# DarylFernandes99/custom-yolo-implmentation

Hardware: AMD Instinct MI355X
Metric: images/sec (640x640 bf16) (higher is better)
Workload: dtype bf16; 1 GPU; preset s (width 32..512, depth 1) 640x640 train step (fwd+DFL/QFL loss+bwd+grad sync+AdamW), COCO-80 synthetic, 32 img/GPU; global_batch=32, parallelism=dp1, hip_graph=True, optimizer_in_graph=True, deterministic_mode=False

## Files before the change

custom-yolo-implmentation_amd/csrc/elementwise.hip:

```cpp
#include "common.h"

namespace {

constexpr int TPB = 256;
constexpr int RS_ROWS = 2;
constexpr int RS_MAXBLK = 256 * 8;

template <typename T> __host__ bool vec_ok(const void* p, long ld, int C) {
    constexpr int V = vec_of<T>::N;
    return (C % V == 0) && (ld % V == 0) && ((reinterpret_cast<uintptr_t>(p) % 16) == 0);
}

template <typename TI, typename TO>
__global__ void k_ncm_to_nhwc(const TI* __restrict__ src, long sn, long sc, long off,
                              TO* __restrict__ dst, int ld, int C, int HW) {
    __shared__ float tile[32][33];
    const int n = blockIdx.z, p0 = blockIdx.x * 32, c0 = blockIdx.y * 32;
    const int tx = threadIdx.x & 31, ty = threadIdx.x >> 5;
    for (int r = ty; r < 32; r += 8) {
        int c = c0 + r, p = p0 + tx;
        tile[r][tx] = (c < C && p < HW) ? to_f<TI>(src[n * sn + c * sc + off + p]) : 0.f;
    }
    __syncthreads();
    for (int r = ty; r < 32; r += 8) {
        int p = p0 + r, c = c0 + tx;
        if (p < HW && c < C) dst[((long)n * HW + p) * ld + c] = from_f<TO>(tile[tx][r]);
    }
}

template <typename TI, typename TO>
__global__ void k_nhwc_to_ncm(const TI* __restrict__ src, int ld, TO* __restrict__ dst, long sn,
                              long sc, long off, int C, int HW) {
    __shared__ float tile[32][33];
    const int n = blockIdx.z, p0 = blockIdx.x * 32, c0 = blockIdx.y * 32;
    const int tx = threadIdx.x & 31, ty = threadIdx.x >> 5;
    for (int r = ty; r < 32; r += 8) {
        int p = p0 + r, c = c0 + tx;
        tile[r][tx] = (p < HW && c < C) ? to_f<TI>(src[((long)n * HW + p) * ld + c]) : 0.f;
    }
    __syncthreads();
    for (int r = ty; r < 32; r += 8) {
        int c = c0 + r, p = p0 + tx;
        if (c < C && p < HW) dst[n * sn + c * sc + off + p] = from_f<TO>(tile[tx][r]);
    }
}

constexpr int HEAD_GROUP = 8;
struct HeadGroup {
    void* t[HEAD_GROUP];
    int ld[HEAD_GROUP], C[HEAD_GROUP], HW[HEAD_GROUP], c_off[HEAD_GROUP], m_off[HEAD_GROUP], tp[HEAD_GROUP];
    int start[HEAD_GROUP + 1];
    int n;
};

template <typename T, bool PACK>
__global__ __launch_bounds__(256) void k_head_group(HeadGroup g, T* __restrict__ preds, long sn, long sc) {
    __shared__ float tile[32][33];
    int bi = 0;
#pragma unroll
    for (int i = 1; i < HEAD_GROUP; ++i)
        if (i < g.n && (int)blockIdx.x >= g.start[i]) bi = i;
    T* x; int ld, C, HW, c_off, m_off, tp, st;
#define HG_PICK(I) case I: x = (T*)g.t[I]; ld = g.ld[I]; C = g.C[I]; HW = g.HW[I]; c_off = g.c_off[I]; m_off = g.m_off[I]; tp = g.tp[I]; st = g.start[I]; break;
    switch (bi) {
        HG_PICK(1) HG_PICK(2) HG_PICK(3) HG_PICK(4) HG_PICK(5) HG_PICK(6) HG_PICK(7)
        default: x = (T*)g.t[0]; ld = g.ld[0]; C = g.C[0]; HW = g.HW[0]; c_off = g.c_off[0]; m_off = g.m_off[0]; tp = g.tp[0]; st = g.start[0]; break;
    }
#undef HG_PICK
    const int tl = (int)blockIdx.x - st;
    const int n = blockIdx.y, p0 = (tl % tp) * 32, c0 = (tl / tp) * 32;
    const int tx = threadIdx.x & 31, ty = threadIdx.x >> 5;
    T* pr = preds + n * sn + (long)c_off * sc + m_off;
    if (PACK) {
        for (int r = ty; r < 32; r += 8) {
            const int p = p0 + r, c = c0 + tx;
            tile[r][tx] = (p < HW && c < C) ? to_f<T>(x[((long)n * HW + p) * ld + c]) : 0.f;
        }
        __syncthreads();
        for (int r = ty; r < 32; r += 8) {
            const int c = c0 + r, p = p0 + tx;
            if (c < C && p < HW) pr[c * sc + p] = from_f<T>(tile[tx][r]);
        }
    } else {
        for (int r = ty; r < 32; r += 8) {
            const int c = c0 + r, p = p0 + tx;
            tile[r][tx] = (c < C && p < HW) ? to_f<T>(pr[c * sc + p]) : 0.f;
        }
        __syncthreads();
        for (int r = ty; r < 32; r += 8) {
            const int p = p0 + r, c = c0 + tx;
            if (p < HW && c < C) x[((long)n * HW + p) * ld + c] = from_f<T>(tile[tx][r]);
        }
    }
}

template <typename T, bool PACK>
__global__ __launch_bounds__(256) void k_head_group_vec(HeadGroup g, T* __restrict__ preds, long sn, long sc) {
    extern __shared__ __attribute__((aligned(16))) unsigned char hg_raw[];
    T* tile = reinterpret_cast<T*>(hg_raw);
    int bi = 0;
#pragma unroll
    for (int i = 1; i < HEAD_GROUP; ++i)
        if (i < g.n && (int)blockIdx.x >= g.start[i]) bi = i;
    T* x; int ld, C, HW, c_off, m_off, st;
#define HG_PICK(I) case I: x = (T*)g.t[I]; ld = g.ld[I]; C = g.C[I]; HW = g.HW[I]; c_off = g.c_off[I]; m_off = g.m_off[I]; st = g.start[I]; break;
    switch (bi) {
        HG_PICK(1) HG_PICK(2) HG_PICK(3) HG_PICK(4) HG_PICK(5) HG_PICK(6) HG_PICK(7)
        default: x = (T*)g.t[0]; ld = g.ld[0]; C = g.C[0]; HW = g.HW[0]; c_off = g.c_off[0]; m_off = g.m_off[0]; st = g.start[0]; break;
    }
#undef HG_PICK
    const int n = blockIdx.y, p0 = ((int)blockIdx.x - st) * 64;
    const int LDT = C + 2, cpr = C / 8;
    T* pr = preds + n * sn + (long)c_off * sc + m_off;
    T* xr = x + ((long)n * HW + p0) * ld;
    const int npx = HW - p0 < 64 ? HW - p0 : 64;
    if (PACK) {
        for (int i = threadIdx.x; i < npx * cpr; i += 256) {
            const int p = i / cpr, ch = (i - p * cpr) * 8;
            const pack_t<T, 8> v = load_raw<T, 8>(xr + (long)p * ld + ch);
#pragma unroll
            for (int e = 0; e < 8; ++e) tile[p * LDT + ch + e] = v.v[e];
        }
        __syncthreads();
        for (int i = threadIdx.x; i < C * (npx / 8); i += 256) {
            const int c = i / (npx / 8), pg = (i - c * (npx / 8)) * 8;
            pack_t<T, 8> v;
#pragma unroll
            for (int e = 0; e < 8; ++e) v.v[e] = tile[(pg + e) * LDT + c];
            *reinterpret_cast<pack_t<T, 8>*>(pr + c * sc + p0 + pg) = v;
        }
    } else {
        for (int i = threadIdx.x; i < C * (npx / 8); i += 256) {
            const int c = i / (npx / 8), pg = (i - c * (npx / 8)) * 8;
            const pack_t<T, 8> v = load_raw<T, 8>(pr + c * sc + p0 + pg);
#pragma unroll
            for (int e = 0; e < 8; ++e) tile[(pg + e) * LDT + c] = v.v[e];
        }
        __syncthreads();
        for (int i = threadIdx.x; i < npx * cpr; i += 256) {
            const int p = i / cpr, ch = (i - p * cpr) * 8;
            pack_t<T, 8> v;
#pragma unroll
            for (int e = 0; e < 8; ++e) v.v[e] = tile[p * LDT + ch + e];
            *reinterpret_cast<pack_t<T, 8>*>(xr + (long)p * ld + ch) = v;
        }
    }
}

template <typename T, int V, bool ACC>
__global__ void k_copy_channels(const T* __restrict__ src, int lds_, T* __restrict__ dst, int ldd,
                                long npix, int cv) {
    long total = npix * cv;
    for (long i = blockIdx.x * (long)blockDim.x + threadIdx.x; i < total; i += (long)gridDim.x * blockDim.x) {
// ... 725 lines not shown

static int launch_reduce(int mode, const void* y, int ldy, const void* dout, int ldd, const float* scale,
                         const float* shift, long npix, int C, int act, int dtype, float* partial, int nblk, hipStream_t st) {
    if (nblk != yolo_reduce_nblk(npix, C)) return YOLO_ERR_ARG;
    YOLO_DISPATCH_T(dtype, {
        bool ok = vec_ok<T>(y, ldy, C) && (mode == 0 || vec_ok<T>(dout, ldd, C));
        PICK_V(T, ok, {
            const RsPlan pl = rs_plan(npix, C / V, false);
            PICK_MODE_ACT(mode, act, hipLaunchKernelGGL((k_channel_reduce<T, V, MODE, ACT>), dim3(nblk, pl.grid.y), dim3(TPB), 0, st,
                                                        (const T*)y, ldy, (const T*)dout, ldd, scale, shift, npix, C, partial, pl.tpr));
        });
    });
    return YOLO_LAUNCH_CHECK();
}

int yolo_bn_stats(const void* y, int ldy, long npix, int C, int dtype, float* partial, int nblk, hipStream_t st) {
    return launch_reduce(0, y, ldy, nullptr, 0, nullptr, nullptr, npix, C, 0, dtype, partial, nblk, st);
}

int yolo_bn_finalize(const float* partial, int nblk, long count, int C, const void* gamma, const void* beta,
                     void* running_mean, void* running_var, float momentum, float eps, float* mean,
                     float* invstd, float* scale, float* shift, int pdtype, int bdtype, hipStream_t st) {
    if (!pdt_ok(pdtype) || !pdt_ok(bdtype)) return YOLO_ERR_DTYPE;
    hipLaunchKernelGGL(k_bn_finalize, dim3(ceil_div(C, FIN_CH)), dim3(FIN_CH * FIN_PARTS), 0, st, partial, nblk, (float)count, C,
                       gamma, beta, running_mean, running_var, momentum, eps, mean, invstd, scale, shift, pdtype, bdtype);
    return YOLO_LAUNCH_CHECK();
}

int yolo_bn_eval_coeffs(const void* gamma, const void* beta, const void* running_mean, const void* running_var,
                        float eps, int C, float* scale, float* shift, int pdtype, int bdtype, hipStream_t st) {
    if (!pdt_ok(pdtype) || !pdt_ok(bdtype)) return YOLO_ERR_DTYPE;
    hipLaunchKernelGGL(k_bn_eval_coeffs, dim3(ceil_div(C, 128)), dim3(128), 0, st, gamma, beta, running_mean, running_var, eps, C,
                       scale, shift, pdtype, bdtype);
    return YOLO_LAUNCH_CHECK();
}

int yolo_sum_finalize(const float* partial, int nblk, int C, float* out, hipStream_t st) {
    hipLaunchKernelGGL(k_sum_finalize, dim3(ceil_div(C, FIN_CH)), dim3(FIN_CH * FIN_PARTS), 0, st, partial, nblk, C, out);
    return YOLO_LAUNCH_CHECK();
}

int yolo_bn_act_fwd(const void* y, int ldy, const float* scale, const float* shift, const void* res, int ldres,
                    void* out, int ldout, long npix, int C, int act, int dtype, hipStream_t st) {
    YOLO_DISPATCH_T(dtype, {
        bool ok = vec_ok<T>(y, ldy, C) && vec_ok<T>(out, ldout, C) && (!res || vec_ok<T>(res, ldres, C));
        PICK_V(T, ok, {
            const RsPlan pl = rs_plan(npix, C / V, false);
            hipLaunchKernelGGL((k_bn_act_fwd<T, V>), pl.grid, dim3(TPB), 0, st, (const T*)y, ldy, scale,
                               shift, (const T*)res, ldres, (T*)out, ldout, npix, C / V, act, pl.tpr);
        });
    });
    return YOLO_LAUNCH_CHECK();
}

int yolo_bn_act_bwd_reduce(const void* dout, int ldd, const void* y, int ldy, const float* scale, const float* shift,
                           const float* mean, const float* invstd, long npix, int C, int act, int dtype,
                           float* partial, int nblk, hipStream_t st) {
    return launch_reduce(1, y, ldy, dout, ldd, scale, shift, npix, C, act, dtype, partial, nblk, st);
}

int yolo_bn_bwd_finalize(const float* partial, int nblk, long count, int C, const void* gamma, const float* mean,
                         const float* invstd, void* dgamma, void* dbeta, float* coef, int pdtype, hipStream_t st) {
    if (!pdt_ok(pdtype)) return YOLO_ERR_DTYPE;
    hipLaunchKernelGGL(k_bn_bwd_finalize, dim3(ceil_div(C, FIN_CH)), dim3(FIN_CH * FIN_PARTS), 0, st, partial, nblk,
                       (float)count, C, gamma, mean, invstd, dgamma, dbeta, coef, pdtype);
    return YOLO_LAUNCH_CHECK();
}

int yolo_bn_act_bwd_apply(const void* dout, int ldd, const void* y, int ldy, const float* scale, const float* shift,
                          const float* mean, const float* invstd, const float* coef, void* dy, int lddy, long npix,
                          int C, int act, int dtype, hipStream_t st) {
    YOLO_DISPATCH_T(dtype, {
        bool ok = vec_ok<T>(y, ldy, C) && vec_ok<T>(dout, ldd, C) && vec_ok<T>(dy, lddy, C);
        PICK_V(T, ok, {
            const RsPlan pl = rs_plan(npix, C / V, false);
            hipLaunchKernelGGL((k_bn_act_bwd_apply<T, V>), pl.grid, dim3(TPB), 5 * pl.tpr * V * sizeof(float), st, (const T*)dout,
                               ldd, (const T*)y, ldy, scale, shift, coef, (T*)dy, lddy, npix, C, act, pl.tpr);
        });
    });
    return YOLO_LAUNCH_CHECK();
}

int yolo_bn_acc_elems(int C) { return BN_REPL * 2 * C; }

static int launch_acc(int mode, const void* y, int ldy, const void* dout, int ldd, const float* scale, const float* shift,
                      long npix, int C, int act, int dtype, float* acc, hipStream_t st) {
    YOLO_DISPATCH_T(dtype, {
        bool ok = vec_ok<T>(y, ldy, C) && (mode == 0 || vec_ok<T>(dout, ldd, C));
        PICK_V(T, ok, {
            const RsPlan pl = rs_plan(npix, C / V, true);
            PICK_MODE_ACT(mode, act, hipLaunchKernelGGL((k_channel_acc<T, V, MODE, ACT>), pl.grid, dim3(TPB), 0, st, (const T*)y, ldy,
                                                        (const T*)dout, ldd, scale, shift, npix, C, acc, pl.tpr));
        });
    });
    return YOLO_LAUNCH_CHECK();
}

int yolo_bn_stats_acc(const void* y, int ldy, long npix, int C, int dtype, float* acc, hipStream_t st) {
    return launch_acc(0, y, ldy, nullptr, 0, nullptr, nullptr, npix, C, 0, dtype, acc, st);
}

int yolo_bn_finalize_acc(const float* acc, long count, int C, const void* gamma, const void* beta, void* running_mean,
                         void* running_var, float momentum, float eps, float* mean, float* invstd, float* scale,
                         float* shift, int pdtype, int bdtype, hipStream_t st) {
    if (!pdt_ok(pdtype) || !pdt_ok(bdtype)) return YOLO_ERR_DTYPE;
    hipLaunchKernelGGL(k_bn_finalize_acc, dim3(ceil_div(C, 64)), dim3(64), 0, st, acc, (float)count, C, gamma, beta,
                       running_mean, running_var, momentum, eps, mean, invstd, scale, shift, pdtype, bdtype);
    return YOLO_LAUNCH_CHECK();
}

int yolo_bn_act_fwd_train(const void* y, int ldy, const float* acc, long count, const void* gamma, const void* beta,
                          void* running_mean, void* running_var, float momentum, float eps, float* mean, float* invstd,
                          float* scale, float* shift, const void* res, int ldres, void* out, int ldout, long npix, int C,
                          int act, int dtype, int pdtype, int bdtype, hipStream_t st) {
    if (!pdt_ok(pdtype) || !pdt_ok(bdtype)) return YOLO_ERR_DTYPE;
    YOLO_DISPATCH_T(dtype, {
        bool ok = vec_ok<T>(y, ldy, C) && vec_ok<T>(out, ldout, C) && (!res || vec_ok<T>(res, ldres, C));
        PICK_V(T, ok, {
            const RsPlan pl = rs_plan(npix, C / V, true);
            PICK_ACT(act, hipLaunchKernelGGL((k_bn_act_fwd_train<T, V, ACT>), pl.grid, dim3(TPB), 2 * pl.tpr * V * sizeof(float), st,
                               (const T*)y, ldy, acc, (float)count, gamma, beta, running_mean, running_var, momentum, eps,
                               mean, invstd, scale, shift, (const T*)res, ldres, (T*)out, ldout, npix, C, pl.tpr, pdtype, bdtype));
        });
    });
    return YOLO_LAUNCH_CHECK();
}

int yolo_bn_bwd_reduce_acc(const void* dout, int ldd, const void* y, int ldy, const float* scale, const float* shift,
                           long npix, int C, int act, int dtype, float* acc, hipStream_t st) {
    return launch_acc(1, y, ldy, dout, ldd, scale, shift, npix, C, act, dtype, acc, st);
}

int yolo_bn_act_bwd_apply_train(const void* dout, int ldd, const void* y, int ldy, const float* scale, const float* shift,
                                const void* gamma, const float* mean, const float* invstd, const float* acc, long count,
                                void* dgamma, void* dbeta, void* dy, int lddy, long npix, int C, int act, int dtype,
                                int pdtype, hipStream_t st) {
    if (!pdt_ok(pdtype)) return YOLO_ERR_DTYPE;
    YOLO_DISPATCH_T(dtype, {
        bool ok = vec_ok<T>(y, ldy, C) && vec_ok<T>(dout, ldd, C) && vec_ok<T>(dy, lddy, C);
        PICK_V(T, ok, {
            const RsPlan pl = rs_plan(npix, C / V, true);
            PICK_ACT(act, hipLaunchKernelGGL((k_bn_act_bwd_apply_train<T, V, ACT>), pl.grid, dim3(TPB), 5 * pl.tpr * V * sizeof(float), st,
                               (const T*)dout, ldd, (const T*)y, ldy, scale, shift, gamma, mean, invstd, acc, (float)count,
                               dgamma, dbeta, (T*)dy, lddy, npix, C, pl.tpr, pdtype));
        });
    });
    return YOLO_LAUNCH_CHECK();
}

int yolo_maxpool5_fwd(const void* x, int ldx, void* out, int ldo, uint8_t* idx, int N, int H, int W, int C,
                      int dtype, hipStream_t st) {
    YOLO_DISPATCH_T(dtype, {
        bool ok = vec_ok<T>(x, ldx, C) && vec_ok<T>(out, ldo, C);
        PICK_V(T, ok, {
            hipLaunchKernelGGL((k_maxpool5_fwd<T, V>), dim3(ew_grid((long)N * H * W * (C / V))), dim3(TPB), 0, st,
                               (const T*)x, ldx, (T*)out, ldo, idx, N, H, W, C);
        });
    });
    return YOLO_LAUNCH_CHECK();
}

int yolo_maxpool5_bwd(const void* dout, int ldd, const uint8_t* idx, void* dx, int ldx, int N, int H, int W, int C,
                      int accumulate, int dtype, hipStream_t st) {
    YOLO_DISPATCH_T(dtype, {
        bool ok = vec_ok<T>(dout, ldd, C) && vec_ok<T>(dx, ldx, C);
        PICK_V(T, ok, {
            int g = ew_grid((long)N * H * W * (C / V));
            if (accumulate)
                hipLaunchKernelGGL((k_maxpool5_bwd<T, V, true>), dim3(g), dim3(TPB), 0, st, (const T*)dout, ldd, idx,
                                   (T*)dx, ldx, N, H, W, C);
            else
                hipLaunchKernelGGL((k_maxpool5_bwd<T, V, false>), dim3(g), dim3(TPB), 0, st, (const T*)dout, ldd, idx,
                                   (T*)dx, ldx, N, H, W, C);
        });
    });
    return YOLO_LAUNCH_CHECK();
}

int yolo_upsample2x_fwd(const void* x, int ldx, void* out, int ldo, int N, int H, int W, int C, int dtype,
                        hipStream_t st) {
    YOLO_DISPATCH_T(dtype, {
        bool ok = vec_ok<T>(x, ldx, C) && vec_ok<T>(out, ldo, C);
        PICK_V(T, ok, {
            hipLaunchKernelGGL((k_upsample2x_fwd<T, V>), dim3(ew_grid((long)N * 4 * H * W * (C / V))), dim3(TPB), 0, st,
                               (const T*)x, ldx, (T*)out, ldo, N, H, W, C);
        });
    });
    return YOLO_LAUNCH_CHECK();
}

int yolo_upsample2x_bwd(const void* dout, int ldd, void* dx, int ldx, int N, int H, int W, int C, int accumulate,
                        int dtype, hipStream_t st) {
    YOLO_DISPATCH_T(dtype, {
        bool ok = vec_ok<T>(dout, ldd, C) && vec_ok<T>(dx, ldx, C);
        PICK_V(T, ok, {
            int g = ew_grid((long)N * H * W * (C / V));
            if (accumulate)
                hipLaunchKernelGGL((k_upsample2x_bwd<T, V, true>), dim3(g), dim3(TPB), 0, st, (const T*)dout, ldd,
                                   (T*)dx, ldx, N, H, W, C);
            else
                hipLaunchKernelGGL((k_upsample2x_bwd<T, V, false>), dim3(g), dim3(TPB), 0, st, (const T*)dout, ldd,
                                   (T*)dx, ldx, N, H, W, C);
        });
    });
    return YOLO_LAUNCH_CHECK();
}

}
```

include/yolo_hip.h:

```cpp
#ifndef YOLO_HIP_H
#define YOLO_HIP_H
#include <stddef.h>
#include <stdint.h>

#ifdef __cplusplus
extern "C" {
#endif

#ifndef __HIP__
typedef struct ihipStream_t* hipStream_t;
#endif

#define YOLO_F32 0
#define YOLO_BF16 1
#define YOLO_F16 2
#define YOLO_ERR_ARG 1001
#define YOLO_ERR_DTYPE 1002
#define YOLO_ACT_IDENTITY 0
#define YOLO_ACT_SILU 1

long yolo_abi_hash(void);

int yolo_memset0(void* p, size_t bytes, hipStream_t st);
int yolo_ncm_to_nhwc(const void* src, int src_dtype, long sn, long sc, long off, void* dst, int dst_dtype, int ld, int N, int C, int HW, hipStream_t st);
int yolo_nhwc_to_ncm(const void* src, int src_dtype, int ld, void* dst, int dst_dtype, long sn, long sc, long off, int N, int C, int HW, hipStream_t st);
int yolo_head_group(int pack, int n, void* const* branches, const int* lds, const int* Cs, const int* HWs, const int* c_offs, const int* m_offs, void* preds, int cp, int M, int N, int dtype, hipStream_t st);
int yolo_copy_channels(const void* src, int ld_src, void* dst, int ld_dst, long npix, int C, int accumulate, int dtype, hipStream_t st);
int yolo_scale_inplace(void* x, long n, int dtype, const float* scale_dev, hipStream_t st);
int yolo_add_n(const void* s0, int ld0, const void* s1, int ld1, const void* s2, int ld2, const void* s3, int ld3, int nsrc, void* dst, int ld_dst, long npix, int C, int dtype, hipStream_t st);

int yolo_conv_kpad(int O, int I, int k, int stride, int mode, int cls);
long yolo_conv_dgrad_wbuf_elems(int O, int I, int k, int stride);
int yolo_conv_pack_weights(const void* w_oihw, int w_dtype, int O, int I, int k, int stride, int mode, void* out, int out_dtype, hipStream_t st);
int yolo_conv_unpack_wgrad(const float* dwp, int O, int I, int k, void* dw_oihw, int dw_dtype, hipStream_t st);
int yolo_pack_job_bytes();
int yolo_pack_job_count(int stride, int mode);
long yolo_pack_job_fill(void* jobs_host, const void* w, int w_dtype, void* out, int out_elem_bytes, int O, int I, int k, int stride, int mode, long start);
long yolo_pack_jobs_finalize(void* jobs_host, int njobs);
int yolo_pack_batched(const void* jobs_dev, int njobs, long nchunks, int out_dtype, hipStream_t st);
int yolo_adamw_job_bytes();
int yolo_adamw_job_fill(void* jobs_host, int index, void* p, int p_dtype, const void* g, int g_dtype, float* m, float* v, long n);
long yolo_adamw_jobs_finalize(void* jobs_host, int njobs);
int yolo_adamw_jobs_set_grads(void* jobs_host, int njobs, const void* const* grads);
int yolo_adamw_step(const void* jobs_dev, int njobs, long nchunks, const double* hyper, float* step, const float* grad_scale, const float* found_inf, hipStream_t st);
int yolo_adamw_job_set_ema(void* jobs_host, int index, float* ema, double* ema_ctl);
int yolo_ema_lerp(const void* jobs_dev, int njobs, long nchunks, const double* ema_ctl, const float* skip_flag, hipStream_t st);
int yolo_adamw_amp_step(const void* jobs_dev, int njobs, long nchunks, const double* hyper, float* step, float* amp_state, int* growth_tracker, float growth_factor, float backoff_factor, int growth_interval, hipStream_t st);
int yolo_grad_sqnorm(const void* jobs_dev, int njobs, long nchunks, float* partials, float* found_inf, hipStream_t st);
int yolo_grad_clip_finalize(const float* partials, long nparts, float* clip_state, const float* grad_scale, hipStream_t st);
int yolo_adamw_clip_step(const void* jobs_dev, int njobs, long nchunks, const double* hyper, float* step, const float* grad_scale, const float* found_inf, const float* clip_state, hipStream_t st);
int yolo_amp_update_scale(float* amp_state, int* growth_tracker, float growth_factor, float backoff_factor, int growth_interval, hipStream_t st);
int yolo_sgd_step(const void* jobs_dev, int njobs, long nchunks, const double* hyper, float* step, const float* grad_scale, const float* found_inf, const float* clip_state, hipStream_t st);
int yolo_sgd_amp_step(const void* jobs_dev, int njobs, long nchunks, const double* hyper, float* step, float* amp_state, int* growth_tracker, float growth_factor, float backoff_factor, int growth_interval, hipStream_t st);
int yolo_copy_job_bytes();
int yolo_copy_job_fill(void* jobs_host, int index, const void* src, int src_dtype, void* dst, int dst_dtype, long n);
long yolo_copy_jobs_finalize(void* jobs_host, int njobs);
int yolo_multi_copy(const void* jobs_dev, int njobs, long nchunks, float scale, hipStream_t st);
int yolo_conv2d_fwd(const void* x, int ldx, const void* wp, const float* bias, void* y, int ldy, float* stats_acc, int N, int H, int W, int Cin, int OH, int OW, int Cout, int k, int stride, int dtype, int algo, hipStream_t st);
int yolo_conv2d_fwd_act(const void* x, int ldx, const void* wp, const float* bias, const void* res, int ldr, void* y, int ldy, int N, int H, int W, int Cin, int OH, int OW, int Cout, int k, int stride, int act, int dtype, hipStream_t st);
int yolo_conv2d_dgrad(const void* dy, int lddy, const void* wb, void* dx, int lddx, int N, int H, int W, int Cin, int OH, int OW, int Cout, int k, int stride, int accumulate, int dtype, int algo, hipStream_t st);
int yolo_conv2d_dgrad_acc2(const void* dy, int lddy, const void* wb, void* dx, int lddx, const void* acc2, int ld2, int N, int H, int W, int Cin, int OH, int OW, int Cout, int k, int stride, int dtype, int algo, hipStream_t st);
long yolo_conv2d_wgrad_ws_elems(const void* x, int ldx, const void* dy, int ldy, int N, int H, int W, int Cin, int OH, int OW, int Cout, int k, int stride, int dtype, int algo);
int yolo_conv2d_wgrad(const void* x, int ldx, const void* dy, int ldy, float* ws, void* dw_oihw, int dw_dtype, int N, int H, int W, int Cin, int OH, int OW, int Cout, int k, int stride, int dtype, int algo, hipStream_t st);
int yolo_conv_tune_set(int bn, int tap_inner, int halo, int dma, int ring, int bm, int nst, int bk);
int yolo_wgrad_tune_set(int to, int ti, int blocks, int min_per);
int yolo_wgrad_tune_pf(int pf);
int yolo_conv_wide_set(int on);
int yolo_conv2d_plan(int N, int H, int W, int Cin, int OH, int OW, int Cout, int k, int stride, int mode, int cls, int dtype);
long yolo_conv2d_wgrad_plan(int N, int H, int W, int Cin, int OH, int OW, int Cout, int k, int stride, int dtype);
int yolo_stem_im2col(const void* img, int img_dtype, void* col, int col_dtype, int N, int H, int W, int OH, int OW, hipStream_t st);
int yolo_stem_pack_weights(const void* w, int w_dtype, int Cout, void* out, int out_dtype, hipStream_t st);
int yolo_stem_unpack_wgrad(const float* dw32, int Cout, void* dw, int dw_dtype, hipStream_t st);
int yolo_stem_conv_eligible(int img_dtype, int dtype, int Cout);
int yolo_stem_conv_fwd(const float* img, const void* wp, void* y, int ldy, float* stats, int N, int H, int W, int OH, int OW, int Cout, const float* bias, int act, int dtype, hipStream_t st);
int yolo_stem_wgrad_slabs();
int yolo_stem_wgrad(const float* img, const void* dy, int ldy, float* partial, void* dw, int dw_dtype, int N, int H, int W, int OH, int OW, int Cout, int dtype, hipStream_t st);
int yolo_dwconv3x3_fwd(const void* x, int ldx, const float* w, void* y, int ldy, int N, int H, int W, int C, int dtype, hipStream_t st);
int yolo_dwconv3x3_fwd_stats(const void* x, int ldx, const float* w, void* y, int ldy, float* stats, int N, int H, int W, int C, int dtype, hipStream_t st);
int yolo_dwconv3x3_fwd_act(const void* x, int ldx, const float* w, const float* bias, void* y, int ldy, int N, int H, int W, int C, int act, int dtype, hipStream_t st);
int yolo_dwconv3x3_dgrad(const void* dy, int lddy, const float* w, void* dx, int lddx, int N, int H, int W, int C, int accumulate, int dtype, hipStream_t st);
int yolo_dw_wgrad_nslab(int N, int H);
int yolo_dwconv3x3_wgrad(const void* x, int ldx, const void* dy, int ldy, float* dw, float* partial, int N, int H, int W, int C, int dtype, hipStream_t st);
int yolo_dw_tune_set(int variant);
int yolo_dw_plan(int N, int H, int W, int C, int field);

int yolo_reduce_nblk(long npix, int C);
int yolo_bn_stats(const void* y, int ldy, long npix, int C, int dtype, float* partial, int nblk, hipStream_t st);
int yolo_bn_finalize(const float* partial, int nblk, long count, int C, const void* gamma, const void* beta, void* running_mean, void* running_var, float momentum, float eps, float* mean, float* invstd, float* scale, float* shift, int pdtype, int bdtype, hipStream_t st);
int yolo_bn_eval_coeffs(const void* gamma, const void* beta, const void* running_mean, const void* running_var, float eps, int C, float* scale, float* shift, int pdtype, int bdtype, hipStream_t st);
int yolo_sum_finalize(const float* partial, int nblk, int C, float* out, hipStream_t st);
int yolo_bn_act_fwd(const void* y, int ldy, const float* scale, const float* shift, const void* res, int ldres, void* out, int ldout, long npix, int C, int act, int dtype, hipStream_t st);
int yolo_bn_act_bwd_reduce(const void* dout, int ldd, const void* y, int ldy, const float* scale, const float* shift, const float* mean, const float* invstd, long npix, int C, int act, int dtype, float* partial, int nblk, hipStream_t st);
int yolo_bn_bwd_finalize(const float* partial, int nblk, long count, int C, const void* gamma, const float* mean, const float* invstd, void* dgamma, void* dbeta, float* coef, int pdtype, hipStream_t st);
int yolo_bn_act_bwd_apply(const void* dout, int ldd, const void* y, int ldy, const float* scale, const float* shift, const float* mean, const float* invstd, const float* coef, void* dy, int lddy, long npix, int C, int act, int dtype, hipStream_t st);
int yolo_bn_acc_elems(int C);
int yolo_bn_stats_acc(const void* y, int ldy, long npix, int C, int dtype, float* acc, hipStream_t st);
int yolo_bn_finalize_acc(const float* acc, long count, int C, const void* gamma, const void* beta, void* running_mean, void* running_var, float momentum, float eps, float* mean, float* invstd, float* scale, float* shift, int pdtype, int bdtype, hipStream_t st);
int yolo_bn_act_fwd_train(const void* y, int ldy, const float* acc, long count, const void* gamma, const void* beta, void* running_mean, void* running_var, float momentum, float eps, float* mean, float* invstd, float* scale, float* shift, const void* res, int ldres, void* out, int ldout, long npix, int C, int act, int dtype, int pdtype, int bdtype, hipStream_t st);
int yolo_bn_bwd_reduce_acc(const void* dout, int ldd, const void* y, int ldy, const float* scale, const float* shift, long npix, int C, int act, int dtype, float* acc, hipStream_t st);
int yolo_bn_act_bwd_apply_train(const void* dout, int ldd, const void* y, int ldy, const float* scale, const float* shift, const void* gamma, const float* mean, const float* invstd, const float* acc, long count, void* dgamma, void* dbeta, void* dy, int lddy, long npix, int C, int act, int dtype, int pdtype, hipStream_t st);

int yolo_maxpool5_fwd(const void* x, int ldx, void* out, int ldo, uint8_t* idx, int N, int H, int W, int C, int dtype, hipStream_t st);
int yolo_maxpool5_bwd(const void* dout, int ldd, const uint8_t* idx, void* dx, int ldx, int N, int H, int W, int C, int accumulate, int dtype, hipStream_t st);
int yolo_upsample2x_fwd(const void* x, int ldx, void* out, int ldo, int N, int H, int W, int C, int dtype, hipStream_t st);
int yolo_upsample2x_bwd(const void* dout, int ldd, void* dx, int ldx, int N, int H, int W, int C, int accumulate, int dtype, hipStream_t st);

size_t yolo_attn_stash_bytes(int N, int T_, int heads, int dtype);
size_t yolo_attn_workspace_bytes(int N, int T_, int heads, int dtype);
size_t yolo_attn_stash_bytes_for(int N, int T, int heads, int dk, int dh, int dtype);
size_t yolo_attn_workspace_bytes_for(int N, int T, int heads, int dk, int dh, int dtype);
int yolo_attn_fwd(const void* qkv, int ldq, void* o, int ldo, void* vp, int ldv, void* stash, void* ws, int N, int T_, int heads, int dk, int dh, float scale, int dtype, hipStream_t st);
int yolo_attn_fwd_nograd(const void* qkv, int ldq, void* o, int ldo, void* vp, int ldv, int N, int T_, int heads, int dk, int dh, float scale, int dtype, hipStream_t st);
int yolo_attn_bwd(const void* qkv, int ldq, const void* o, int ldo, const void* d_o, int lddo, const void* d_vp, int lddv, const void* stash, void* ws, void* dqkv, int lddq, int N, int T_, int heads, int dk, int dh, float scale, int dtype, hipStream_t st);

size_t yolo_loss_workspace_bytes(int N, int A, int G);
int yolo_loss_dfl_qfl(const void* preds, const void* anchors, const void* strides, int dtype, int N, int nc, int A, const float* gt, const int* gt_off, const int* gt_img, int G, float lambda_dfl, float lambda_cls, void* dpreds, float* out, void* workspace, const float* grad_scale, hipStream_t st);

size_t yolo_loss_tal_workspace_bytes(int N, int A, int G);
int yolo_loss_tal(const void* preds, const void* anchors, const void* strides, int dtype, int N, int nc, int A, const float* gt, const int* gt_off, const int* gt_img, int G, int topk, float alpha, float beta, float lambda_box, float lambda_cls, float lambda_dfl, void* dpreds, float* out, void* workspace, const float* grad_scale, hipStream_t st);

int yolo_bbox_iou(const float* box1, const float* box2, int M, float* iou, const float* g, float* db1, float* db2, hipStream_t st);
int yolo_quality_focal_loss(const float* pred, const float* target, int M, int C, float beta, float* out, const float* g, float* dpred, float* dtarget, hipStream_t st);
int yolo_distribution_focal_loss(const float* pred_dist, const float* target_val, int M, int C, float* out, const float* g, float* dpred, float* dtarget, hipStream_t st);

int yolo_head_decode(const void* preds, const void* anchors, const void* strides, void* y, int N, int nc, int A, int dtype, hipStream_t st);
int yolo_dfl_expect(const void* x, void* y, int B, int A, int dtype, hipStream_t st);
int yolo_nms_capacity(int M, int nc, int multi_label);
size_t yolo_nms_workspace_bytes(int bs, int M, int nc, int multi_label);
int yolo_nms(const void* y, int dtype, int bs, int nc, int M, float conf_thres, float iou_thres, const int* classes, int n_classes, int agnostic, int multi_label, int max_det, float* out, int* out_count, int* status, void* workspace, hipStream_t st);

size_t yolo_val_workspace_bytes(int N, int M, int top_k);
int yolo_val_select(const void* y, int dtype, int N, int nc, int M, float conf, int top_k, float* out, int* out_count, void* workspace, hipStream_t st);
int yolo_val_match(const float* pred, const int* count, int N, int top_k, const float* gt, const int* gt_off, double iou_thr, int nc, int skip_empty_gt, long long* counters, int* status, hipStream_t st);

int yolo_prep_image_bytes();
int yolo_prep_image_fill(void* table_host, int index, long off, int H, int W, int flip, int o0, int o1, int o2, int o3, float brightness, float contrast, float saturation, float hue);
int yolo_image_prep(const void* src, const void* table_dev, int N, int S, int jitter, void* stage, float* means, void* out, int out_dtype, float m0, float m1, float m2, float s0, float s1, float s2, hipStream_t st);
int yolo_mosaic_tile_bytes();
int yolo_mosaic_tile_fill(void* table_host, int image, int tile, long off, int H, int W, int flip, int tw, int th, int x0, int y0, int cx, int cy);
int yolo_image_prep_mosaic(const void* src, const void* tiles_dev, const void* table_dev, int N, int S, int fill, int jitter, void* stage, float* means, void* out, int out_dtype, float m0, float m1, float m2, float s0, float s1, float s2, hipStream_t st);

int yolo_selftest_tr16(const void* tile_in, void* out, hipStream_t st);
int yolo_selftest_glds(const void* in128x16, void* out64x16, hipStream_t st);
int yolo_selftest_dma_vs_xlane(const void* pattern4k, int blocks, int iters, int spam, void* errors, void* sink, hipStream_t st);
int yolo_selftest_dma_order(const void* src, long src_bytes, int blocks, int kind, void* errors2, hipStream_t st);
int yolo_selftest_ring_vs_xlane(const void* src, int steps, int blocks, int spam, void* errors, void* sink, hipStream_t st);
int yolo_selftest_permlane16(const void* in64, void* out128, hipStream_t st);
int yolo_selftest_grid_barrier(void* counters, int blocks, int rounds, int tree, int* timed_out, hipStream_t st);

#ifdef __cplusplus
}
#endif
#endif
```

Baseline: 3103 images/s.

## Add LDS-tiled separable maxpool5 forward and backward kernels for SPPF

Adds LDS-tiled kernels for the 5x5 maxpool used in SPPF. Each workgroup stages a spatial tile plus halo and a group of channel packets into LDS. The forward pass is made separable: a row max with argmax, then a column max, with the combined index written out. The backward pass gathers gradients from the staged dout and index tile instead of making per-tap global reads. The new path is on by default when the plan fits in LDS, which trades fewer redundant global reads for large LDS use and possibly lower occupancy.

```diff
diff --git a/custom-yolo-implmentation_amd/csrc/elementwise.hip b/custom-yolo-implmentation_amd/csrc/elementwise.hip
--- a/custom-yolo-implmentation_amd/csrc/elementwise.hip
+++ b/custom-yolo-implmentation_amd/csrc/elementwise.hip
@@ -1,4 +1,5 @@
 #include "common.h"
+#include "pool.h"
 
 namespace {
 
@@ -1030,6 +1031,7 @@
                       int dtype, hipStream_t st) {
     YOLO_DISPATCH_T(dtype, {
         bool ok = vec_ok<T>(x, ldx, C) && vec_ok<T>(out, ldo, C);
+        if (pool_takes_tile(N, H, W, C, dtype, ok, false)) return pool_tile_fwd(x, ldx, out, ldo, idx, N, H, W, C, dtype, st);
         PICK_V(T, ok, {
             hipLaunchKernelGGL((k_maxpool5_fwd<T, V>), dim3(ew_grid((long)N * H * W * (C / V))), dim3(TPB), 0, st,
                                (const T*)x, ldx, (T*)out, ldo, idx, N, H, W, C);
@@ -1042,6 +1044,8 @@
                       int accumulate, int dtype, hipStream_t st) {
     YOLO_DISPATCH_T(dtype, {
         bool ok = vec_ok<T>(dout, ldd, C) && vec_ok<T>(dx, ldx, C);
+        if (pool_takes_tile(N, H, W, C, dtype, ok, true))
+            return pool_tile_bwd(dout, ldd, idx, dx, ldx, N, H, W, C, accumulate, dtype, st);
         PICK_V(T, ok, {
             int g = ew_grid((long)N * H * W * (C / V));
             if (accumulate)
@@ -1053,6 +1057,19 @@
         });
     });
     return YOLO_LAUNCH_CHECK();
+}
+
+int yolo_pool_tune_set(int variant, int packets, int pixels) { return pool_tune_set(variant, packets, pixels); }
+
+int yolo_pool_plan(int N, int H, int W, int C, int dtype, int aligned, int field) {
+    if (N < 1 || H < 1 || W < 1 || C < 1 || (dtype != YOLO_F32 && dtype != YOLO_BF16 && dtype != YOLO_F16)) return -1;
+    const int V = dtype == YOLO_F32 ? 4 : 8;
+    const bool vec = aligned != 0 && C % V == 0;
+    if (field == 0 || field == 1) return pool_takes_tile(N, H, W, C, dtype, vec, field == 1) ? 1 : 2;
+    PoolPlan p;
+    if (!vec || !pool_plan(N, H, W, C, V, p)) return 0;
+    const long f[] = {p.P, p.ngrp, p.bw, p.ncb, p.bh, p.nb, p.th, p.tw, p.lds_fwd, p.lds_bwd, p.wgs};
+    return field >= 2 && field <= 12 ? (int)f[field - 2] : -1;
 }
 
 int yolo_upsample2x_fwd(const void* x, int ldx, void* out, int ldo, int N, int H, int W, int C, int dtype,
diff --git a/custom-yolo-implmentation_amd/csrc/pool.h b/custom-yolo-implmentation_amd/csrc/pool.h
--- /dev/null
+++ b/custom-yolo-implmentation_amd/csrc/pool.h
@@ -0,0 +1,19 @@
+#pragma once
+#include "common.h"
+
+struct PoolPlan {
+    int P, ngrp;
+    int bw, ncb, bh, nb;
+    int th, tw;
+    long lds_fwd, lds_bwd;
+    long wgs;
+};
+bool pool_plan(int N, int H, int W, int C, int V, PoolPlan& p);
+
+int pool_tune_set(int variant, int packets, int pixels);
+
+bool pool_takes_tile(int N, int H, int W, int C, int dtype, bool vec, bool backward);
+
+int pool_tile_fwd(const void* x, int ldx, void* out, int ldo, uint8_t* idx, int N, int H, int W, int C, int dtype, hipStream_t st);
+int pool_tile_bwd(const void* dout, int ldd, const uint8_t* idx, void* dx, int ldx, int N, int H, int W, int C, int accumulate,
+                  int dtype, hipStream_t st);
diff --git a/custom-yolo-implmentation_amd/csrc/pool.hip b/custom-yolo-implmentation_amd/csrc/pool.hip
--- /dev/null
+++ b/custom-yolo-implmentation_amd/csrc/pool.hip
@@ -0,0 +1,361 @@
+#include "pool.h"
+
+#include <cstdlib>
+#include <cstring>
+
+namespace {
+
+constexpr int PT = 256;
+constexpr int PL = 4;
+constexpr int POOL_PIX = 512;
+constexpr long POOL_LDS_MAX = 160 * 1024;
+
+struct PoolGeom { int N, H, W, C, P, bh, nb, bw, ncb, th, tw; };
+
+struct PoolTile { int n, h0, h1, w0, w1, r0, r1, c0, c1, pk0, np; };
+
+struct PoolDiv { int d, m; };
+__device__ __forceinline__ PoolDiv pool_div(int d) { return PoolDiv{d, ((1 << 20) + d - 1) / d}; }
+__device__ __forceinline__ void pool_divmod(int n, const PoolDiv& f, int& q, int& r) {
+    q = (int)(__umul24((unsigned)n, (unsigned)f.m) >> 20);
+    r = n - q * f.d;
+}
+
+template <int V>
+__device__ __forceinline__ PoolTile pool_tile(const PoolGeom& g) {
+    PoolTile t;
+    int s = (int)blockIdx.x;
+    const int cb = s % g.ncb; s /= g.ncb;
+    const int band = s % g.nb;
+    t.n = s / g.nb;
+    t.h0 = band * g.bh; t.h1 = min(t.h0 + g.bh, g.H);
+    t.w0 = cb * g.bw;   t.w1 = min(t.w0 + g.bw, g.W);
+    t.r0 = max(t.h0 - 2, 0); t.r1 = min(t.h1 + 2, g.H);
+    t.c0 = max(t.w0 - 2, 0); t.c1 = min(t.w1 + 2, g.W);
+    t.pk0 = (int)blockIdx.y * g.P;
+    t.np = min(g.P, g.C / V - t.pk0);
+    return t;
+}
+
+template <typename E, int V>
+__device__ __forceinline__ void pool_stage(const E* __restrict__ src, long ld, const PoolGeom& g, const PoolTile& t,
+                                           pack_t<E, V>* __restrict__ tile) {
+    const int twa = t.c1 - t.c0, cnt = (t.r1 - t.r0) * twa * t.np;
+    const PoolDiv dnp = pool_div(t.np), dtw = pool_div(twa);
+    for (int b = (int)threadIdx.x; b < cnt; b += PL * PT) {
+        pack_t<E, V> raw[PL];
+#pragma unroll
+        for (int u = 0; u < PL; ++u) {
+            const int e = min(b + u * PT, cnt - 1);
+            int pk, px, tc, tr;
+            pool_divmod(e, dnp, px, pk);
+            pool_divmod(px, dtw, tr, tc);
+            raw[u] = load_raw<E, V>(src + (((long)t.n * g.H + t.r0 + tr) * g.W + t.c0 + tc) * ld + (long)(t.pk0 + pk) * V);
+        }
+#pragma unroll
+        for (int u = 0; u < PL; ++u)
+            if (b + u * PT < cnt) tile[b + u * PT] = raw[u];
+    }
+}
+
+template <typename T, int V>
+__global__ __launch_bounds__(PT) void k_maxpool5_fwd_tile(const T* __restrict__ x, int ldx, T* __restrict__ out, int ldo,
+                                                          uint8_t* __restrict__ idx, PoolGeom g) {
+    extern __shared__ __attribute__((aligned(16))) unsigned char pool_lds[];
+    const PoolTile t = pool_tile<V>(g);
+    const int tha = t.r1 - t.r0, twa = t.c1 - t.c0, bha = t.h1 - t.h0, bwa = t.w1 - t.w0, np = t.np;
+    pack_t<T, V>* tile = reinterpret_cast<pack_t<T, V>*>(pool_lds);
+    pack_t<T, V>* rmax = tile + g.th * g.tw * g.P;
+    pack_t<uint8_t, V>* rkw = reinterpret_cast<pack_t<uint8_t, V>*>(rmax + g.th * g.bw * g.P);
+    pool_stage<T, V>(x, ldx, g, t, tile);
+    __syncthreads();
+    const int nrow = tha * bwa * np;
+    const PoolDiv dnp = pool_div(np), dbw = pool_div(bwa);
+    for (int i = (int)threadIdx.x; i < nrow; i += PT) {
+        int pk, q, wo, tr;
+        pool_divmod(i, dnp, q, pk);
+        pool_divmod(q, dbw, tr, wo);
+        const int w = t.w0 + wo;
+        pack_t<T, V> raw[5];
+#pragma unroll
+        for (int kw = 0; kw < 5; ++kw) {
+            const int wc = min(max(w + kw - 2, 0), g.W - 1);
+            raw[kw] = tile[(tr * twa + wc - t.c0) * np + pk];
+        }
+        float best[V];
+        pack_t<uint8_t, V> bk;
+#pragma unroll
+        for (int j = 0; j < V; ++j) { best[j] = -INFINITY; bk.v[j] = 0; }
+        bool first = true;
+#pragma unroll
+        for (int kw = 0; kw < 5; ++kw) {
+            const int ww = w + kw - 2;
+            if (ww < 0 || ww >= g.W) continue;
+            float a[V];
+            unpack<T, V>(raw[kw], a);
+#pragma unroll
+            for (int j = 0; j < V; ++j)
+                if (a[j] > best[j] || a[j] != a[j] || first) { best[j] = a[j]; bk.v[j] = (uint8_t)kw; }
+            first = false;
+        }
+        pack_t<T, V> bv;
+#pragma unroll
+        for (int j = 0; j < V; ++j) bv.v[j] = from_f<T>(best[j]);
+        rmax[i] = bv;
+        rkw[i] = bk;
+    }
+    __syncthreads();
+    const int nout = bha * bwa * np;
+    for (int i = (int)threadIdx.x; i < nout; i += PT) {
+        int pk, q, wo, ho;
+        pool_divmod(i, dnp, q, pk);
+        pool_divmod(q, dbw, ho, wo);
+        const int h = t.h0 + ho;
+        pack_t<T, V> rv[5];
+        pack_t<uint8_t, V> rk[5];
+#pragma unroll
+        for (int kh = 0; kh < 5; ++kh) {
+            const int hc = min(max(h + kh - 2, 0), g.H - 1);
+            const int a = ((hc - t.r0) * bwa + wo) * np + pk;
+            rv[kh] = rmax[a];
+            rk[kh] = rkw[a];
+        }
+        float best[V];
+        pack_t<uint8_t, V> bi;
+#pragma unroll
+        for (int j = 0; j < V; ++j) { best[j] = -INFINITY; bi.v[j] = 0; }
+        bool first = true;
+#pragma unroll
+        for (int kh = 0; kh < 5; ++kh) {
+            const int hh = h + kh - 2;
+            if (hh < 0 || hh >= g.H) continue;
+            float a[V];
+            unpack<T, V>(rv[kh], a);
+#pragma unroll
+            for (int j = 0; j < V; ++j)
+                if (a[j] > best[j] || a[j] != a[j] || first) { best[j] = a[j]; bi.v[j] = (uint8_t)(kh * 5 + rk[kh].v[j]); }
+            first = false;
+        }
+        const long p = ((long)t.n * g.H + h) * g.W + t.w0 + wo;
+        store_pack<T, V>(out + p * ldo + (long)(t.pk0 + pk) * V, best);
+        *reinterpret_cast<pack_t<uint8_t, V>*>(idx + p * g.C + (long)(t.pk0 + pk) * V) = bi;
+    }
+}
+
+typedef float pool_f4 __attribute__((ext_vector_type(4)));
+typedef float pool_f2 __attribute__((ext_vector_type(2)));
+template <int V> struct alignas(V) PoolIdx { uint32_t w[V / 4]; };
+
+template <typename T, int V>
+__device__ __forceinline__ void pool_stage_bwd(const T* __restrict__ dout, long ldd, const uint8_t* __restrict__ idx, const PoolGeom& g,
+                                               const PoolTile& t, pool_f4* __restrict__ dtile, int plane, PoolIdx<V>* __restrict__ itile) {
+    const int twa = t.c1 - t.c0, cnt = (t.r1 - t.r0) * twa * t.np;
+    const PoolDiv dnp = pool_div(t.np), dtw = pool_div(twa);
+    for (int b = (int)threadIdx.x; b < cnt; b += PL * PT) {
+        pack_t<T, V> raw[PL];
+        PoolIdx<V> ri[PL];
+#pragma unroll
+        for (int u = 0; u < PL; ++u) {
+            const int e = min(b + u * PT, cnt - 1);
+            int pk, px, tc, tr;
+            pool_divmod(e, dnp, px, pk);
+            pool_divmod(px, dtw, tr, tc);
+            const long q = ((long)t.n * g.H + t.r0 + tr) * g.W + t.c0 + tc;
+            raw[u] = load_raw<T, V>(dout + q * ldd + (long)(t.pk0 + pk) * V);
+            ri[u] = *reinterpret_cast<const PoolIdx<V>*>(idx + q * g.C + (long)(t.pk0 + pk) * V);
+        }
+#pragma unroll
+        for (int u = 0; u < PL; ++u) {
+            const int e = b + u * PT;
+            if (e >= cnt) continue;
+            float d[V];
+            unpack<T, V>(raw[u], d);
+#pragma unroll
+            for (int k = 0; k < V / 4; ++k) dtile[k * plane + e] = pool_f4{d[4 * k], d[4 * k + 1], d[4 * k + 2], d[4 * k + 3]};
+            itile[e] = ri[u];
+        }
+    }
+}
+
+template <typename T, int V, bool ACC>
+__device__ __forceinline__ void pool_bwd_item(int i, const pack_t<T, V>& acc, const pool_f4* __restrict__ dtile, int plane,
+                                              const PoolIdx<V>* __restrict__ itile, T* __restrict__ dx, int ldx, const PoolGeom& g,
+                                              const PoolTile& t, const PoolDiv& dnp, const PoolDiv& dbw) {
+    const int twa = t.c1 - t.c0, np = t.np;
+    int pk, q, wo, ho;
+    pool_divmod(i, dnp, q, pk);
+    pool_divmod(q, dbw, ho, wo);
+    const int h = t.h0 + ho, w = t.w0 + wo;
+    pool_f2 s[V / 2];
+#pragma unroll
+    for (int j = 0; j < V / 2; ++j) s[j] = pool_f2{0.f, 0.f};
+#pragma unroll
+    for (int kh = 0; kh < 5; ++kh) {
+        const int oh = h - kh + 2;
+        const bool rok = oh >= 0 && oh < g.H;
+        const int oc = min(max(oh, 0), g.H - 1);
+        pool_f4 raw[5][V / 4];
+        PoolIdx<V> ri[5];
+#pragma unroll
+        for (int kw = 0; kw < 5; ++kw) {
+            const int wc = min(max(w - kw + 2, 0), g.W - 1);
+            const int a = ((oc - t.r0) * twa + wc - t.c0) * np + pk;
+#pragma unroll
+            for (int k = 0; k < V / 4; ++k) raw[kw][k] = dtile[k * plane + a];
+            ri[kw] = itile[a];
+        }
+#pragma unroll
+        for (int kw = 0; kw < 5; ++kw) {
+            const int ow = w - kw + 2;
+            if (!(rok && ow >= 0 && ow < g.W)) continue;
+#pragma unroll
+            for (int j = 0; j < V / 2; ++j) {
+                const uint32_t wd = ri[kw].w[j / 2];
+                const bool m0 = ((wd >> (16 * (j & 1))) & 0xffu) == (uint32_t)(kh * 5 + kw);
+                const bool m1 = ((wd >> (16 * (j & 1) + 8)) & 0xffu) == (uint32_t)(kh * 5 + kw);
+                const pool_f4 d4 = raw[kw][j / 2];
+                const float d0 = (j & 1) ? d4.z : d4.x, d1 = (j & 1) ? d4.w : d4.y;
+                s[j] += pool_f2{m0 ? d0 : 0.f, m1 ? d1 : 0.f};
+            }
+        }
+    }
+    float r[V];
+#pragma unroll
+    for (int j = 0; j < V / 2; ++j) { r[2 * j] = s[j].x; r[2 * j + 1] = s[j].y; }
+    if (ACC) {
+        float b[V];
+        unpack<T, V>(acc, b);
+#pragma unroll
+        for (int j = 0; j < V; ++j) r[j] += b[j];
+    }
+    const long p = ((long)t.n * g.H + h) * g.W + w;
+    store_pack<T, V>(dx + p * ldx + (long)(t.pk0 + pk) * V, r);
+}
+
+template <typename T, int V>
+__device__ __forceinline__ pack_t<T, V> pool_bwd_acc(int i, const T* __restrict__ dx, int ldx, const PoolGeom& g, const PoolTile& t,
+                                                     const PoolDiv& dnp, const PoolDiv& dbw) {
+    int pk, q, wo, ho;
+    pool_divmod(i, dnp, q, pk);
+    pool_divmod(q, dbw, ho, wo);
+    const long p = ((long)t.n * g.H + t.h0 + ho) * g.W + t.w0 + wo;
+    return load_raw<T, V>(dx + p * ldx + (long)(t.pk0 + pk) * V);
+}
+
+template <typename T, int V, bool ACC>
+__global__ __launch_bounds__(PT) void k_maxpool5_bwd_tile(const T* __restrict__ dout, int ldd, const uint8_t* __restrict__ idx,
+                                                          T* __restrict__ dx, int ldx, PoolGeom g) {
+    extern __shared__ __attribute__((aligned(16))) unsigned char pool_lds[];
+    const PoolTile t = pool_tile<V>(g);
+    const int plane = g.th * g.tw * g.P;
+    pool_f4* dtile = reinterpret_cast<pool_f4*>(pool_lds);
+    PoolIdx<V>* itile = reinterpret_cast<PoolIdx<V>*>(dtile + (V / 4) * plane);
+    const int nout = (t.h1 - t.h0) * (t.w1 - t.w0) * t.np;
+    const PoolDiv dnp = pool_div(t.np), dbw = pool_div(t.w1 - t.w0);
+    pack_t<T, V> pre[PL] = {};
+    if (ACC) {
+#pragma unroll
+        for (int u = 0; u < PL; ++u) pre[u] = pool_bwd_acc<T, V>(min((int)threadIdx.x + u * PT, nout - 1), dx, ldx, g, t, dnp, dbw);
+    }
+    pool_stage_bwd<T, V>(dout, ldd, idx, g, t, dtile, plane, itile);
+    __syncthreads();
+#pragma unroll
+    for (int u = 0; u < PL; ++u) {
+        const int i = (int)threadIdx.x + u * PT;
+        if (i < nout) pool_bwd_item<T, V, ACC>(i, pre[u], dtile, plane, itile, dx, ldx, g, t, dnp, dbw);
+    }
+    for (int i = (int)threadIdx.x + PL * PT; i < nout; i += PT) {
+        pack_t<T, V> a = {};
+        if (ACC) a = pool_bwd_acc<T, V>(i, dx, ldx, g, t, dnp, dbw);
+        pool_bwd_item<T, V, ACC>(i, a, dtile, plane, itile, dx, ldx, g, t, dnp, dbw);
+    }
+}
+
+struct PoolTune { int variant, packets, pixels; };
+PoolTune& pool_tune() {
+    static PoolTune v = [] {
+        const char* e = getenv("YOLO_POOL_KERNEL");
+        return PoolTune{e == nullptr ? 0 : strcmp(e, "taps") == 0 ? 1 : strcmp(e, "tile") == 0 ? 2 : 0, 0, 0};
+    }();
+    return v;
+}
+
+PoolGeom pool_geom(const PoolPlan& p, int N, int H, int W, int C) {
+    return PoolGeom{N, H, W, C, p.P, p.bh, p.nb, p.bw, p.ncb, p.th, p.tw};
+}
+
+}
+
+bool pool_plan(int N, int H, int W, int C, int V, PoolPlan& p) {
+    if (N < 1 || H < 1 || W < 1 || C < V || C % V != 0) return false;
+    const int cv = C / V;
+    p.ncb = ceil_div(W, 32);
+    p.bw = ceil_div(W, p.ncb);
+    p.ncb = ceil_div(W, p.bw);
+    p.tw = p.bw + 4 < W ? p.bw + 4 : W;
+    const int pix = pool_tune().pixels > 0 ? pool_tune().pixels : POOL_PIX;
+    const int th_max = pix / p.tw;
+    if (H <= th_max) { p.nb = 1; p.bh = H; }
+    else {
+        p.nb = ceil_div(H, th_max - 4);
+        p.bh = ceil_div(H, p.nb);
+        p.nb = ceil_div(H, p.bh);
+    }
+    p.th = p.bh + 4 < H ? p.bh + 4 : H;
+    const int tuned = pool_tune().packets;
+    p.P = tuned > 0 ? tuned : ((long)N * p.nb * p.ncb * ceil_div(cv, 2) >= 1024 ? 2 : 1);
+    if (p.P > cv) p.P = cv;
+    for (;;) {
+        p.lds_fwd = (long)p.th * p.tw * p.P * 16 + (long)p.th * p.bw * p.P * (16 + V);
+        p.lds_bwd = (long)p.th * p.tw * p.P * (4 * V + V);
+        if ((p.lds_fwd <= POOL_LDS_MAX && p.lds_bwd <= POOL_LDS_MAX) || p.P == 1) break;
+        p.P /= 2;
+    }
+    p.ngrp = ceil_div(cv, p.P);
+    p.wgs = (long)N * p.nb * p.ncb * p.ngrp;
+    return p.lds_fwd <= POOL_LDS_MAX && p.lds_bwd <= POOL_LDS_MAX && (long)N * p.nb * p.ncb < (1L << 31) && p.ngrp < 65536;
+}
+
+int pool_tune_set(int variant, int packets, int pixels) {
+    if (variant < 0 || variant > 2 || packets < 0 || packets > 8 || (pixels != 0 && (pixels < 256 || pixels > POOL_PIX))) return YOLO_ERR_ARG;
+    pool_tune() = PoolTune{variant, packets, pixels};
+    return YOLO_OK;
+}
+
+bool pool_takes_tile(int N, int H, int W, int C, int dtype, bool vec, bool backward) {
+    (void)backward;
+    const int v = pool_tune().variant;
+    if (!vec || v == 1) return false;
+    if (dtype != YOLO_F32 && dtype != YOLO_BF16 && dtype != YOLO_F16) return false;
+    PoolPlan p;
+    return pool_plan(N, H, W, C, dtype == YOLO_F32 ? 4 : 8, p);
+}
+
+int pool_tile_fwd(const void* x, int ldx, void* out, int ldo, uint8_t* idx, int N, int H, int W, int C, int dtype, hipStream_t st) {
+    YOLO_DISPATCH_T(dtype, {
+        constexpr int V = vec_of<T>::N;
+        PoolPlan p;
+        if (!pool_plan(N, H, W, C, V, p)) return YOLO_ERR_ARG;
+        return launch_dyn_lds<k_maxpool5_fwd_tile<T, V>>(dim3((unsigned)((long)N * p.nb * p.ncb), (unsigned)p.ngrp), dim3(PT),
+                                                         (size_t)p.lds_fwd, st, (const T*)x, ldx, (T*)out, ldo, idx,
+                                                         pool_geom(p, N, H, W, C));
+    });
+    return YOLO_ERR_DTYPE;
+}
+
+int pool_tile_bwd(const void* dout, int ldd, const uint8_t* idx, void* dx, int ldx, int N, int H, int W, int C, int accumulate,
+                  int dtype, hipStream_t st) {
+    YOLO_DISPATCH_T(dtype, {
+        constexpr int V = vec_of<T>::N;
+        PoolPlan p;
+        if (!pool_plan(N, H, W, C, V, p)) return YOLO_ERR_ARG;
+        const dim3 grid((unsigned)((long)N * p.nb * p.ncb), (unsigned)p.ngrp);
+        const PoolGeom g = pool_geom(p, N, H, W, C);
+        if (accumulate)
+            return launch_dyn_lds<k_maxpool5_bwd_tile<T, V, true>>(grid, dim3(PT), (size_t)p.lds_bwd, st, (const T*)dout, ldd, idx,
+                                                                   (T*)dx, ldx, g);
+        return launch_dyn_lds<k_maxpool5_bwd_tile<T, V, false>>(grid, dim3(PT), (size_t)p.lds_bwd, st, (const T*)dout, ldd, idx,
+                                                                (T*)dx, ldx, g);
+    });
+    return YOLO_ERR_DTYPE;
+}
diff --git a/include/yolo_hip.h b/include/yolo_hip.h
--- a/include/yolo_hip.h
+++ b/include/yolo_hip.h
@@ -102,6 +102,8 @@
 
 int yolo_maxpool5_fwd(const void* x, int ldx, void* out, int ldo, uint8_t* idx, int N, int H, int W, int C, int dtype, hipStream_t st);
 int yolo_maxpool5_bwd(const void* dout, int ldd, const uint8_t* idx, void* dx, int ldx, int N, int H, int W, int C, int accumulate, int dtype, hipStream_t st);
+int yolo_pool_tune_set(int variant, int packets, int pixels);
+int yolo_pool_plan(int N, int H, int W, int C, int dtype, int aligned, int field);
 int yolo_upsample2x_fwd(const void* x, int ldx, void* out, int ldo, int N, int H, int W, int C, int dtype, hipStream_t st);
 int yolo_upsample2x_bwd(const void* dout, int ldd, void* dx, int ldx, int N, int H, int W, int C, int accumulate, int dtype, hipStream_t st);
 
```

Result: no change. 3102 images/s (median of 2 runs) (-0.0%).
